# pachterlab/kallisto

Hardware: NVIDIA H100
Metric: paired reads/sec quant (higher is better)
Workload: dtype u64/f64

## Files before the change

kallisto_b200/csrc/kernels_align.cu:

```cuda
#include "kb_device.cuh"
#include "kb_dict.cuh"
#include "kernels.hpp"

#ifndef KB_MATCH_MIN_BLOCKS
#define KB_MATCH_MIN_BLOCKS 3
#endif
#ifdef KB_MATCH_STATS
#include <cstdio>
#endif

namespace kb {

#ifdef KB_MATCH_STATS
enum : int {
  MS_WARP_ITERS, MS_SERVICE_ROUNDS, MS_LANE_ITERS, MS_CHAIN_ITERS,
  MS_MAIN_HIT, MS_MAIN_MISS_FILTER, MS_MAIN_MISS_SLOT, MS_JUMP, MS_MIDDLE, MS_BACKOFF, MS_COLLISION,
  MS_CYCLES_LOOKUP, MS_CYCLES_SERVICE,
  MS_CYCLES_KEY, MS_CYCLES_WAIT, MS_CYCLES_STEP,
  MS_RUN_HIST, MS_N = MS_RUN_HIST + 9
};
__device__ unsigned long long kb_match_stats[MS_N];
static const char* const kMatchStatNames[MS_N] = {
  "warp_iters", "service_rounds", "lane_iters", "chain_iters",
  "main_hit", "main_miss_filter", "main_miss_slot", "jump", "middle", "backoff", "collision",
  "cycles_lookup", "cycles_service", "cycles_key", "cycles_wait", "cycles_step",
  "run_1", "run_2", "run_3", "run_4", "run_5_8", "run_9_16", "run_17_32", "run_33_64", "run_65_"};
__device__ __forceinline__ int run_bin(int n) {
  return n <= 4 ? n - 1 : (n <= 8 ? 4 : (n <= 16 ? 5 : (n <= 32 ? 6 : (n <= 64 ? 7 : 8))));
}
#define KB_MS(i, n) (ms[i] += (unsigned long long)(n))
#define KB_MS_ONLY(x) x
#else
#define KB_MS(i, n) ((void)0)
#define KB_MS_ONLY(x)
#endif

namespace {

__device__ __forceinline__ int32_t ld_relaxed_s32(const int32_t* p) {
  int32_t v;
  asm volatile("ld.relaxed.gpu.global.s32 %0, [%1];" : "=r"(v) : "l"(p) : "memory");
  return v;
}
__device__ __forceinline__ void ld256_nc(const void* p, uint32_t (&w)[8]) {
  asm volatile("ld.global.nc.v4.b32 {%0,%1,%2,%3}, [%8]; ld.global.nc.v4.b32 {%4,%5,%6,%7}, [%8+16];"
               : "=r"(w[0]), "=r"(w[1]), "=r"(w[2]), "=r"(w[3]), "=r"(w[4]), "=r"(w[5]), "=r"(w[6]), "=r"(w[7])
               : "l"(p));
}
struct ReadView {
  const uint32_t* bw;
  const uint32_t* gmask;
  int n_mask;
  int stride;
  int len;
  int k;
  bool has_invalid;

  __device__ __forceinline__ uint64_t kmer(int p) const {
    const int w = p >> 4, s = (p & 15) * 2;
    uint64_t x = (uint64_t)bw[w * stride] << 32;
    if (s + 2 * k > 32) x |= bw[(w + 1) * stride];
    x <<= s;
    if (s + 2 * k > 64) x |= (uint64_t)(bw[(w + 2) * stride] >> (32 - s));
    return x >> (64 - 2 * k);
  }
  __device__ __forceinline__ int next_valid(int p) const {
    if (!has_invalid) return p <= len - k ? p : -1;
    const uint64_t wmask = (1ULL << k) - 1;
    while (p <= len - k) {
      const int w = p >> 5, s = p & 31;
      const uint64_t lo = __ldg(gmask + w);
      const uint64_t hi = (w + 1 < n_mask) ? __ldg(gmask + w + 1) : 0xFFFFFFFFu;
      const uint64_t x = (((hi << 32) | lo) >> s) & wmask;
      if (x == 0) return p;
      p += 64 - __clzll((long long)x);
    }
    return -1;
  }
};

__device__ __forceinline__ uint64_t tuple_hash(const uint32_t* w, int n, int stride) {
  uint64_t h = 0x243F6A8885A308D3ULL ^ (uint64_t)n;
  for (int i = 0; i < n; ++i) h = kb_mix64(h ^ ((uint64_t)w[i * stride] + 0x9E3779B97F4A7C15ULL * (i + 1)));
  return h;
}

__device__ __forceinline__ int32_t memo2_lookup(const DevDict& dd, uint32_t e0, uint32_t e1) {
  const unsigned long long key = ((unsigned long long)e0 << 32) | e1;
  uint64_t s = kb_mix64(key) & dd.m2_mask;
  for (;;) {
    const unsigned long long kk = __ldcg(&dd.m2[s].key);
    if (kk == key) return ld_relaxed_s32(&dd.m2[s].val);
    if (kk == ~0ULL) return KB_H_NOTREADY;
    s = (s + 1) & dd.m2_mask;
  }
}
__device__ __forceinline__ bool tuple_equal(const DevDict& dd, uint32_t toff, const uint32_t* w, int n, int stride) {
  const uint32_t* t = dd.tpool + toff;
  bool eq = __ldcg(t) == (uint32_t)n;
  for (int i = 0; eq && i < n; ++i) eq = __ldcg(t + 1 + i) == w[i * stride];
  return eq;
}
__device__ __forceinline__ int32_t memon_lookup(const DevDict& dd, const uint32_t* w, int n, int stride) {
  const uint64_t th = tuple_hash(w, n, stride);
  const uint32_t tag = (uint32_t)(th >> 32);
  uint64_t s = th & dd.mn_mask;
  for (;;) {
    const unsigned long long word = ld_acquire_u64(&dd.mn_key[s]);
    if (word == ~0ULL) return KB_H_NOTREADY;
    if ((uint32_t)(word >> 32) == tag && tuple_equal(dd, (uint32_t)word, w, n, stride)) return ld_relaxed_s32(&dd.mn_val[s]);
    s = (s + 1) & dd.mn_mask;
  }
}

__device__ __forceinline__ void read_span(const BatchArgs& ba, uint32_t ridx, const uint8_t*& base, uint64_t& off, int& len) {
  base = ba.bases;
  const uint32_t* offs = ba.off;
  uint32_t i = ridx;
  if (ba.bases2) {
    i = ridx >> 1;
    if (ridx & 1) { base = ba.bases2; offs = ba.off2; }
  }
  if (offs) {
    const uint32_t o0 = offs[i], o1 = offs[i + 1];
    off = o0;
    len = (int)(o1 - o0);
  } else {
    off = (uint64_t)i * ba.fixed_len;
    len = (int)ba.fixed_len;
  }
  const bool second = ba.paired && (ridx & 1);
  uint32_t st = second ? ba.start2 : ba.start;
  if (ba.notag && ba.notag[ba.paired ? (ridx >> 1) : ridx]) st = second ? ba.alt_start2 : ba.alt_start;
  if (st) {
    off += st;
    len -= (int)st;
    if (len < 0) len = 0;
  }
  if (ba.skip && ba.skip[ba.paired ? (ridx >> 1) : ridx]) len = 0;
}

enum : int {
  S_MAIN = 0, S_JUMP = 1, S_MIDDLE = 2, S_BACKOFF = 3,
  S_FIN = 4,
  S_EMPTY = 5
};
enum : int { C_BLK = 0, C_DS = 1, C_POS = 2, C_NP = 3, C_H2U = 4, C_H2E = 5, C_P2 = 6, C_P3 = 7, C_DIST = 8, C_HU = 9, C_HE = 10 };
static_assert(C_HE + 1 == KB_CHAIN_WORDS, "match_lane_words counts every cold word of a chain");

}

__global__ void __launch_bounds__(256) pack_kernel(BatchArgs ba, uint32_t n_reads, uint32_t* out) {
  const uint32_t gid = blockIdx.x * blockDim.x + threadIdx.x;
  const uint32_t nb = ba.nb;
  if (gid >= n_reads * nb) return;
  const uint32_t r = gid / nb, w = gid - r * nb;
  uint64_t off;
  int len;
  const uint8_t* src_bases;
  read_span(ba, r, src_bases, off, len);
  const int base = (int)w * 32;
  uint32_t hi = 0, lo = 0, inv32 = ~0u;
  if (base < len) {
    const int n = min(32, len - base);
    const uint64_t a = off + (uint64_t)base;
    const uint32_t* wp = reinterpret_cast<const uint32_t*>(src_bases + (a & ~3ull));
    const int sh = (int)(a & 3) * 8;
    const int last = ((int)(a & 3) + n - 1) >> 2;
    uint32_t wd[9];
#pragma unroll
    for (int q = 0; q < 9; ++q) wd[q] = __ldg(wp + min(q, last));
    uint32_t d[8], pr[8];
#pragma unroll
    for (int q = 0; q < 8; ++q) {
      const uint32_t four = __funnelshift_r(wd[q], wd[q + 1], sh);
      uint32_t x = (four >> 1) & 0x03030303u;
      const uint32_t y = (x | (x >> 4)) & 0x00330033u;
      d[q] = (four & 0xDFDFDFDFu) ^ __byte_perm(0x47544341u, 0u, y | (y >> 8));
      x ^= (x >> 1) & 0x01010101u;
      pr[q] = x * 0x40100401u;
    }
    hi = __byte_perm(__byte_perm(pr[3], pr[2], 0x0073u), __byte_perm(pr[1], pr[0], 0x0073u), 0x5410u);
    lo = __byte_perm(__byte_perm(pr[7], pr[6], 0x0073u), __byte_perm(pr[5], pr[4], 0x0073u), 0x5410u);
    const bool full = (n == 32);
    uint32_t any = full ? (d[0] | d[1] | d[2] | d[3] | d[4] | d[5] | d[6] | d[7]) : 1u;
    inv32 = 0;
    if (any) {
      const int ng = (n + 3) >> 2;
#pragma unroll
      for (int q = 0; q < 8; ++q) {
        if (q >= ng) break;
        uint32_t t = (d[q] & 0x7F7F7F7Fu) + 0x7F7F7F7Fu;
        t = (t | d[q]) & 0x80808080u;
        inv32 |= (((t >> 7) * 0x01020408u) >> 24) << (4 * q);
      }
    }
    if (!full) {
      inv32 |= ~0u << n;
      if (n > 16) lo &= ~0u << (64 - 2 * n);
      else { lo = 0; if (n < 16) hi &= ~0u << (32 - 2 * n); }
    }
  }
  uint32_t* dst = out + (size_t)r * ba.pstride;
  reinterpret_cast<uint2*>(dst)[w] = make_uint2(lo, hi);
  dst[2 * nb + w] = inv32;
  for (uint32_t j = 3 * nb + w; j < ba.pstride; j += nb) dst[j] = ~0u;
}

__global__ void __launch_bounds__(256) dlist_scan_kernel(DevIndex ix, BatchArgs ba, uint32_t n_reads) {
  const uint64_t gid = (uint64_t)blockIdx.x * blockDim.x + threadIdx.x;
  const uint32_t nb = ba.nb;
  if (gid >= (uint64_t)n_reads * nb) return;
  const uint32_t r = (uint32_t)(gid / nb), w = (uint32_t)(gid % nb);
  const uint32_t frag = ba.paired ? (r >> 1) : r;
  uint64_t off;
  int len;
  const uint8_t* unused;
  read_span(ba, r, unused, off, len);
  const int k = ix.k;
  const int p0 = (int)w * 32;
  if (len < k || p0 > len - k) return;
  const uint32_t* pk = ba.packed + (size_t)r * ba.pstride;
  const unsigned long long* bw = reinterpret_cast<const unsigned long long*>(pk);
  const unsigned long long w0 = bw[w], w1 = (w + 1 < nb) ? bw[w + 1] : 0ull;
  const unsigned long long inv = (unsigned long long)pk[2 * nb + w] | ((w + 1 < nb) ? ((unsigned long long)pk[2 * nb + w + 1] << 32) : 0xFFFFFFFF00000000ull);
  const unsigned long long wmask = (1ull << k) - 1;
  for (int j = 0; j < 32; ++j) {
    const int p = p0 + j;
    if (p > len - k) break;
    if ((inv >> j) & wmask) continue;
    unsigned long long x = w0 << (2 * j);
    if (j) x |= w1 >> (64 - 2 * j);
    const uint64_t fwd = x >> (64 - 2 * k);
    const uint64_t rc = kb_revcomp(fwd, k);
    const uint64_t canon = fwd < rc ? fwd : rc;
    uint64_t h = kb_mix64(canon) & ix.dfk_mask;
    for (;;) {
      const unsigned long long key = __ldg(ix.dfk + h);
      if (key == canon) { ba.skip_w[frag] = 1; return; }
      if (key == KB_EMPTY_KEY) break;
      h = (h + 1) & ix.dfk_mask;
    }
  }
}

__global__ void __launch_bounds__(256, KB_MATCH_MIN_BLOCKS) match_kernel(DevIndex ix, DevDict dd, BatchArgs ba) {
  extern __shared__ uint32_t smem[];
  const int tid = threadIdx.x, nt = blockDim.x;
  const unsigned lane = tid & 31;
  const int nb = (int)ba.nb, nw = 2 * nb;
  const int k = ix.k;
  uint32_t* elist = smem + tid;
  uint32_t* cold = elist + (size_t)KB_MAX_E * nt;
  uint32_t* s_bw = cold + (size_t)2 * KB_CHAIN_WORDS * nt;
  uint32_t* spill = ba.spill + ((size_t)blockIdx.x * nt + tid) * KB_SPILL;
  static_assert(C_BLK < C_POS && C_DS < C_POS && C_POS == 2 && C_NP == C_POS + 1 && C_HE == KB_CHAIN_WORDS - 1,
                "a tuple grown by 6 words past KB_MAX_E overwrites exactly the first-hit words of both chains");
  auto cw = [&](int w, int c) -> uint32_t& { return cold[(size_t)(2 * w + c) * nt]; };

  const uint32_t n_warps = (gridDim.x * nt) >> 5;
  const uint32_t gw = (blockIdx.x * nt + tid) >> 5;
  const uint32_t chunk = (ba.n_frag + n_warps - 1) / n_warps;
  uint32_t next = min(ba.n_frag, gw * chunk);
  const uint32_t end = min(ba.n_frag, next + chunk);
  const int n_mates = ba.paired ? 2 : 1;
  const int n_chunks = (int)(ba.pstride >> 3);

  __shared__ unsigned long long s_tot[3];
  if (tid < 3) s_tot[tid] = 0;
  __syncthreads();

  uint32_t frag = 0;
  int n_e = 0;
  bool overflow = false;
  unsigned inv_flags = 0;
  int st[2] = {S_EMPTY, S_EMPTY};
  int p[2] = {-1, -1}, len[2] = {0, 0};
  bool need_prep[2] = {false, false}, is_canon[2] = {false, false};
  bool hv[2] = {false, false}, hs[2] = {false, false};
  uint64_t canon[2] = {0, 0};
  uint32_t slot[2] = {0, 0};
  const uint32_t slot_mask = (uint32_t)ix.mask;
  uint32_t pv = 0;
#ifdef KB_MATCH_STATS
  unsigned long long ms[MS_N] = {};
  int run[2] = {0, 0};
  long long t_mark = clock64();
  long long t_step = -1;
  auto end_run = [&](int c) { if (run[c] > 0) { KB_MS(MS_RUN_HIST + run_bin(run[c]), 1); run[c] = 0; } };
#endif
  auto view = [&](int c) {
    ReadView rv;
    rv.bw = s_bw + (size_t)c * nw * nt;
    rv.gmask = ba.packed + (size_t)(ba.paired ? 2 * frag + c : frag) * ba.pstride + nw;
    rv.n_mask = nb;
    rv.stride = nt;
    rv.len = len[c];
    rv.k = k;
    rv.has_invalid = ((inv_flags >> c) & 1u) != 0;
    return rv;
  };

  KB_MS_ONLY(bool in_service = true;)
  for (;;) {
#ifdef KB_MATCH_STATS
    {
      const long long t_now = clock64();
      KB_MS(in_service ? MS_CYCLES_SERVICE : MS_CYCLES_LOOKUP, t_now - t_mark);
      if (t_step >= 0) KB_MS(MS_CYCLES_STEP, t_now - t_step);
      t_mark = t_now;
      t_step = -1;
    }
#endif
    const bool done = st[0] == S_FIN && st[1] == S_FIN;
    const unsigned fin = __ballot_sync(0xFFFFFFFFu, done);
    const unsigned idle = fin | __ballot_sync(0xFFFFFFFFu, st[0] == S_EMPTY);
    const bool work_left = next < end;
    if (idle == 0xFFFFFFFFu && fin == 0 && !work_left) break;
    KB_MS_ONLY(in_service = false;)
    if (idle == 0xFFFFFFFFu || (work_left && __popc(idle) >= ba.refill_min)) {
      KB_MS(MS_SERVICE_ROUNDS, 1);
      KB_MS_ONLY(in_service = true;)
      if (done) {
        bool memo_hit = false;
        const bool v0 = hv[0], s0 = hs[0], v1 = hv[1], s1 = hs[1];
        uint32_t f_blk[2], f_ds[2], f_pos[2];
#pragma unroll
        for (int c = 0; c < 2; ++c) { f_blk[c] = cw(C_BLK, c); f_ds[c] = cw(C_DS, c); f_pos[c] = cw(C_POS, c); }
        bool mapped = v0 || v1;
        if ((v0 && !s0) || (v1 && !s1)) mapped = false;
        if (mapped && n_e == 0) mapped = false;
        int32_t handle = KB_H_UNMAPPED;
        if (mapped) {
          const bool want_fp = ba.fp_fl >= 0 && (!ba.paired || !v0 || !v1);
          const bool stranded = ba.strand_mode != 0;
          uint32_t xs0 = 0xFFFFFFFFu, xs1 = 0xFFFFFFFFu;
          if (stranded) {
            xs0 = v0 ? (f_blk[0] * 2u + (f_ds[0] >> 31)) : 0xFFFFFFFFu;
            xs1 = v1 ? (f_blk[1] * 2u + (f_ds[1] >> 31)) : 0xFFFFFFFFu;
            if (ba.notag && ba.notag[frag]) xs0 = xs1 = 0xFFFFFFFFu;
          }
          const uint32_t x_blk = v1 ? f_blk[1] : f_blk[0], x_ds = v1 ? f_ds[1] : f_ds[0], x_pos = v1 ? f_pos[1] : f_pos[0];
          const uint32_t xf0 = x_blk;
          const uint32_t xf1 = x_ds >> 31;
          const uint32_t xf2 = x_pos;
          const uint32_t xf3 = x_ds & 0x7FFFFFFFu;
          const int nx = (stranded ? 2 : 0) + (want_fp ? 4 : 0);
          auto put_extras = [&](uint32_t* dst, int at, int st) {
            if (stranded) { dst[at * st] = xs0; dst[(at + 1) * st] = xs1; at += 2; }
            if (want_fp) { dst[at * st] = xf0; dst[(at + 1) * st] = xf1; dst[(at + 2) * st] = xf2; dst[(at + 3) * st] = xf3; }
          };
          if (overflow) {
            atomicOr(dd.error, KB_DEVERR_E_OVERFLOW);
          } else if (n_e > KB_MAX_E) {
            auto E = [&](int i) -> uint32_t { return i < KB_MAX_E ? elist[i * nt] : spill[i - KB_MAX_E]; };
            auto S = [&](int i, uint32_t x) { if (i < KB_MAX_E) elist[i * nt] = x; else spill[i - KB_MAX_E] = x; };
            for (int i = 1; i < n_e; ++i) {
              const uint32_t x = E(i);
              int j = i - 1;
              while (j >= 0 && E(j) > x) { S(j + 1, E(j)); --j; }
              S(j + 1, x);
            }
            const uint32_t q = atomicAdd(ba.qbig_count, 1u);
            if (q >= ba.qbig_cap) {
              atomicOr(dd.error, KB_DEVERR_E_OVERFLOW);
            } else {
              uint32_t* e = ba.qbig_entries + (size_t)q * KB_QBIG_STRIDE;
              e[0] = frag;
              e[1] = (uint32_t)(n_e + nx) | (want_fp ? 0x80000000u : 0u) | 0x40000000u;
              for (int i = 0; i < n_e; ++i) e[2 + i] = E(i);
              put_extras(e + 2, n_e, 1);
              handle = KB_H_PENDING;
            }
          } else {
            for (int i = 1; i < n_e; ++i) {
              const uint32_t x = elist[i * nt];
              int j = i - 1;
              while (j >= 0 && elist[j * nt] > x) { elist[(j + 1) * nt] = elist[j * nt]; --j; }
              elist[(j + 1) * nt] = x;
            }
            if (ba.strand_mode == 0 && n_e == 1 && !want_fp) {
              handle = (int32_t)elist[0];
            } else {
              const int n = n_e + nx;
              int32_t r;
              if (ba.strand_mode == 0 && n_e == 2 && !want_fp) {
                r = memo2_lookup(dd, elist[0], elist[nt]);
              } else {
                put_extras(elist, n_e, nt);
                r = want_fp ? KB_H_NOTREADY : memon_lookup(dd, elist, n, nt);
              }
              if (r == KB_H_NOTREADY) {
                handle = KB_H_PENDING;
                const uint32_t q = atomicAdd(ba.q_count, 1u);
                uint32_t* e = ba.q_entries + (size_t)q * KB_Q_STRIDE;
                e[0] = frag;
                e[1] = (uint32_t)n | (want_fp ? 0x80000000u : 0u);
                for (int i = 0; i < n; ++i) e[2 + i] = elist[i * nt];
              } else {
                handle = r;
                memo_hit = true;
              }
            }
          }
        }
        ba.handle_out[frag] = handle;
        if (ba.tl_out) {
          uint16_t tl = 0;
          if (ba.paired && v0 && v1) {
            int q[2];
            bool strand[2];
#pragma unroll
            for (int c = 0; c < 2; ++c) {
              const int d = (int)(f_ds[c] & 0x7FFFFFFFu);
              strand[c] = (f_ds[c] >> 31) != 0;
              q[c] = strand[c] ? d - (int)f_pos[c] : d + k + (int)f_pos[c];
            }
            if (f_blk[0] == f_blk[1] && strand[0] != strand[1]) {
              const int d = q[0] > q[1] ? q[0] - q[1] : q[1] - q[0];
              if (d > 0 && d < 1000) tl = (uint16_t)d;
            }
          }
          if (ba.notag && !ba.notag[frag]) tl = 0;
          ba.tl_out[frag] = tl;
        }
        if (ba.first_hit) ba.first_hit[frag] = v0 ? f_blk[0] * 2u + (f_ds[0] >> 31) : 0xFFFFFFFFu;
        const unsigned grp = __match_any_sync(fin, handle);
        const uint32_t fmin = __reduce_min_sync(grp, frag);
        if (handle >= 0 && !ba.no_count && lane == (unsigned)(__ffs(grp) - 1)) {
          atomicAdd(&dd.count[handle], (uint32_t)__popc(grp));
          atomicMin(&dd.first[handle], (unsigned long long)(ba.frag_base + fmin));
        }
        const uint32_t r_probes = __reduce_add_sync(fin, pv & 0xFFFFu), r_visits = __reduce_add_sync(fin, pv >> 16);
        const uint32_t r_memo = __popc(__ballot_sync(fin, memo_hit));
        pv = 0;
        if (lane == (unsigned)(__ffs(fin) - 1)) {
          atomicAdd(&s_tot[0], (unsigned long long)r_probes);
          atomicAdd(&s_tot[1], (unsigned long long)r_visits);
          if (r_memo) atomicAdd(&s_tot[2], (unsigned long long)r_memo);
        }
        st[0] = st[1] = S_EMPTY;
      }
      __syncwarp();
      {
        const bool is_idle = (idle >> lane) & 1u;
        const uint32_t rank = __popc(idle & ((1u << lane) - 1));
        const uint32_t avail = end - next;
        if (is_idle && rank < avail) {
          const uint32_t fidx = next + rank;
          unsigned inv = 0;
#pragma unroll
          for (int mt = 0; mt < 2; ++mt) {
            len[mt] = 0;
            if (mt >= n_mates) continue;
            const uint32_t ridx = ba.paired ? 2 * fidx + mt : fidx;
            const uint8_t* unused_base;
            uint64_t unused_off;
            int l;
            read_span(ba, ridx, unused_base, unused_off, l);
            if (l > nb * 32) l = nb * 32;
            len[mt] = l;
            const uint32_t* src = ba.packed + (size_t)ridx * ba.pstride;
            uint32_t* dbw = s_bw + (size_t)mt * nw * nt;
            uint32_t bad = 0;
            for (int c = 0; c < n_chunks; ++c) {
              uint32_t v[8];
              ld256_nc(src + c * 8, v);
#pragma unroll
              for (int i = 0; i < 8; ++i) {
                const int g = c * 8 + i;
                if (g < nw) {
                  dbw[(g ^ 1) * nt] = v[i];
                } else if (g < nw + nb) {
                  const int first = (g - nw) * 32;
                  const uint32_t in_read = l >= first + 32 ? 0xFFFFFFFFu : (l > first ? ((1u << (l - first)) - 1u) : 0u);
                  bad |= v[i] & in_read;
                }
              }
            }
            if (bad) inv |= 1u << mt;
          }
          frag = fidx;
          n_e = 0;
          overflow = false;
          inv_flags = inv;
#pragma unroll
          for (int c = 0; c < 2; ++c) {
            hv[c] = hs[c] = false;
            need_prep[c] = true;
            st[c] = S_FIN;
            if (c < n_mates) {
              p[c] = view(c).next_valid(0);
              if (p[c] >= 0) st[c] = S_MAIN;
            }
          }
        }
        const uint32_t n_idle = __popc(idle);
        next += n_idle < avail ? n_idle : avail;
      }
      continue;
    }
    const bool live[2] = {st[0] <= S_BACKOFF, st[1] <= S_BACKOFF};
    KB_MS(MS_WARP_ITERS, 1);
    if (live[0] || live[1]) {
      KB_MS(MS_LANE_ITERS, 1);
      uint32_t fword[2] = {0xFFFFFFFFu, 0xFFFFFFFFu}, fbit[2] = {0, 0};
#pragma unroll
      for (int c = 0; c < 2; ++c) {
        if (live[c] && need_prep[c]) {
          const bool filtered = st[c] == S_MAIN || st[c] == S_BACKOFF;
          const int pq = filtered ? p[c] : (int)cw(st[c] == S_JUMP ? C_P2 : C_P3, c);
          const uint64_t fwd = view(c).kmer(pq);
          const uint64_t rc = kb_revcomp(fwd, k);
          is_canon[c] = fwd < rc;
          canon[c] = is_canon[c] ? fwd : rc;
          const uint64_t hsh = kb_mix64(canon[c]);
          slot[c] = (uint32_t)hsh & slot_mask;
          need_prep[c] = false;
          ++pv;
          if (ix.filter && filtered) {
            const uint32_t fidx = (uint32_t)(hsh >> 32) & ix.filter_mask;
            fword[c] = __ldg(ix.filter + (fidx >> 5));
            fbit[c] = fidx & 31;
          }
        }
      }
#ifdef KB_MATCH_STATS
      const long long t_key = clock64();
#endif
      uint32_t v[2][8];
#pragma unroll
      for (int c = 0; c < 2; ++c) {
        if (live[c] && ((fword[c] >> fbit[c]) & 1u)) {
          ld256_nc(ix.slots + slot[c], v[c]);
          pv += 0x10000u;
        } else {
          v[c][0] = v[c][1] = 0xFFFFFFFFu;
        }
      }
#ifdef KB_MATCH_STATS
      {
        long long t_wait = t_key;
        if (((v[0][0] ^ v[0][1]) ^ 3u * (v[1][0] ^ v[1][1])) != 0x0BADF00Du) t_wait = clock64();
        KB_MS(MS_CYCLES_KEY, t_key - t_mark);
        KB_MS(MS_CYCLES_WAIT, t_wait - t_key);
        t_step = t_wait;
      }
#endif
#pragma unroll
      for (int c = 0; c < 2; ++c) {
        if (!live[c]) continue;
        KB_MS(MS_CHAIN_ITERS, 1);
        const uint64_t key = (uint64_t)v[c][0] | ((uint64_t)v[c][1] << 32);
        if (key != canon[c] && key != KB_EMPTY_KEY) {
          slot[c] = (slot[c] + 1) & slot_mask;
          KB_MS(MS_COLLISION, 1);
          continue;
        }
        const bool f = key == canon[c];
#ifdef KB_MATCH_STATS
        if (st[c] == S_MAIN) {
          if (f) { KB_MS(MS_MAIN_HIT, 1); end_run(c); }
          else { KB_MS(((fword[c] >> fbit[c]) & 1u) ? MS_MAIN_MISS_SLOT : MS_MAIN_MISS_FILTER, 1); ++run[c]; }
        } else {
          KB_MS(st[c] == S_JUMP ? MS_JUMP : (st[c] == S_MIDDLE ? MS_MIDDLE : MS_BACKOFF), 1);
        }
#endif
        const uint32_t r_unitig = v[c][2], r_ec = v[c][4];
        const bool r_strand = (is_canon[c] == ((v[c][5] >> 31) != 0));
        const int l = len[c];
        const ReadView rv = view(c);
        bool push = false, end_chain = false, to_backoff = false;
        int nv_from = -1;
        if (st[c] == S_MAIN) {
          if (!f) {
            nv_from = p[c] + 1;
          } else {
            push = true;
            const int r_dist = (int)(v[c][5] & 0x7FFFFFFFu);
            const int off = r_dist - (int)v[c][6], blen = (int)(v[c][7] - v[c][6]);
            const int dist = r_strand ? (blen - 1 - off) : off;
            if (dist >= 2) {
              const int np = (p[c] + dist >= l - k) ? (l - k) : (p[c] + dist);
              const int p2 = rv.next_valid(np);
              if (p2 < 0) {
                end_chain = true;
              } else {
                cw(C_NP, c) = (uint32_t)np;
                cw(C_P2, c) = (uint32_t)p2;
                cw(C_DIST, c) = (uint32_t)dist;
                cw(C_HU, c) = r_unitig; cw(C_HE, c) = r_ec;
                st[c] = S_JUMP;
                need_prep[c] = true;
              }
            } else {
              nv_from = p[c] + 1;
            }
          }
        } else if (st[c] == S_JUMP) {
          const bool found2 = !f || (cw(C_HU, c) == r_unitig && cw(C_HE, c) == r_ec);
          const int dist = (int)cw(C_DIST, c);
          const int found2pos = !f ? p[c] : p[c] + dist;
          if (found2) {
            if (found2pos >= l - k) end_chain = true;
            else nv_from = (int)cw(C_P2, c) + 1;
          } else {
            cw(C_H2U, c) = r_unitig; cw(C_H2E, c) = r_ec;
            if (dist > 4) {
              const int middlePos = (p[c] + (int)cw(C_NP, c)) / 2;
              const int p3 = rv.next_valid(middlePos);
              if (p3 >= 0) { cw(C_P3, c) = (uint32_t)p3; st[c] = S_MIDDLE; need_prep[c] = true; }
              else to_backoff = true;
            } else {
              to_backoff = true;
            }
          }
        } else if (st[c] == S_MIDDLE) {
          const bool foundMiddle = f && ((cw(C_HU, c) == r_unitig && cw(C_HE, c) == r_ec) ||
                                         (cw(C_H2U, c) == r_unitig && cw(C_H2E, c) == r_ec));
          if (foundMiddle) {
            push = true;
            if ((int)cw(C_NP, c) >= l - k) end_chain = true;
            else nv_from = (int)cw(C_P2, c) + 1;
          } else {
            to_backoff = true;
          }
        } else {
          push = f;
          nv_from = p[c] + 1;
        }
        if (push) {
          if (!hv[c]) {
            hv[c] = true;
            cw(C_BLK, c) = v[c][3];
            cw(C_DS, c) = (v[c][5] & 0x7FFFFFFFu) | (r_strand ? 0x80000000u : 0u);
            cw(C_POS, c) = (uint32_t)p[c];
          }
          if (r_ec != ba.empty_ec) {
            hs[c] = true;
            bool dup = false;
            const int n_sh = n_e < KB_MAX_E ? n_e : KB_MAX_E;
            for (int i = 0; i < n_sh; ++i) dup |= (elist[i * nt] == r_ec);
            for (int i = KB_MAX_E; i < n_e; ++i) dup |= (spill[i - KB_MAX_E] == r_ec);
            if (!dup) {
              if (n_e < KB_MAX_E) { elist[n_e * nt] = r_ec; ++n_e; }
              else if (n_e < KB_MAX_E + KB_SPILL) { spill[n_e - KB_MAX_E] = r_ec; ++n_e; }
              else overflow = true;
            }
          }
        }
        if (to_backoff) nv_from = p[c] + 1;
        if (nv_from >= 0) {
          p[c] = rv.next_valid(nv_from);
          if (p[c] < 0) end_chain = true;
          else { st[c] = to_backoff ? S_BACKOFF : S_MAIN; need_prep[c] = true; }
        }
        if (end_chain) st[c] = S_FIN;
        KB_MS_ONLY(if (st[c] == S_FIN) end_run(c);)
      }
    }
  }
  __syncthreads();
  if (tid < 3 && s_tot[tid]) atomicAdd(&dd.stats[tid == 0 ? 0 : (tid == 1 ? 3 : 2)], s_tot[tid]);
#ifdef KB_MATCH_STATS
  for (int i = 0; i < MS_N; ++i) {
    const bool per_warp = i == MS_WARP_ITERS || i == MS_SERVICE_ROUNDS || i == MS_CYCLES_LOOKUP || i == MS_CYCLES_SERVICE;
    unsigned long long x = ms[i];
    if (!per_warp)
      for (int o = 16; o > 0; o >>= 1) x += __shfl_xor_sync(0xFFFFFFFFu, x, o);
    if (lane == 0 && x) atomicAdd(&kb_match_stats[i], x);
  }
#endif
}

template <int G>
__global__ void __launch_bounds__(128, 8) resolve_kernel(DevIndex ix, DevDict dd, BatchArgs ba, ResolveArgs ra) {
  const unsigned lane = threadIdx.x & (G - 1);
  const unsigned gmask = group_mask<G>(threadIdx.x & 31);
  const unsigned gshift = (threadIdx.x & 31) & ~(unsigned)(G - 1);
  const uint32_t warp = (blockIdx.x * blockDim.x + threadIdx.x) / G;
  if (warp >= ra.n_warps) return;
  uint32_t* scratch = ra.scratch + (size_t)warp * ra.scratch_stride;
  const uint32_t* pool = dd.pool;

  for (int pass = 0; pass < 2; ++pass) {
  const uint32_t nq = pass == 0 ? *ba.q_count : min(*ba.qbig_count, ba.qbig_cap);
  const uint32_t* entries = pass == 0 ? ba.q_entries : ba.qbig_entries;
  const size_t stride = pass == 0 ? (size_t)KB_Q_STRIDE : (size_t)KB_QBIG_STRIDE;
  if (warp == 0 && lane == 0 && nq) atomicAdd(&dd.stats[1], (unsigned long long)nq);
  for (uint32_t q = warp; q < nq; q += ra.n_warps) {
    const uint32_t* e = entries + (size_t)q * stride;
    const uint32_t f = e[0];
    const bool has_fp = (e[1] >> 31) != 0;
    const bool no_memo = has_fp || ((e[1] >> 30) & 1u) != 0;
    const int n = (int)(e[1] & 0xFFFFu);
    const uint32_t* w = e + 2;
    const bool stranded = ba.strand_mode != 0;
    const int n_e = n - (stranded ? 2 : 0) - (has_fp ? 4 : 0);
    const bool use_m2 = (!stranded && !no_memo && n_e == 2);

    int32_t handle = KB_H_NOTREADY;
    if (lane == 0 && !no_memo) handle = use_m2 ? memo2_lookup(dd, w[0], w[1]) : memon_lookup(dd, w, n, 1);
    handle = __shfl_sync(gmask, handle, 0, G);

    if (handle == KB_H_NOTREADY) {
      int sm = 0;
      uint32_t sm_len = (uint32_t)((dd.dslots[w[0]] >> 32) & 0xFFFFFFu);
      for (int j = 1; j < n_e; ++j) {
        const uint32_t len = (uint32_t)((dd.dslots[w[j]] >> 32) & 0xFFFFFFu);
        if (len < sm_len) { sm_len = len; sm = j; }
      }
      const uint32_t* A = pool + (uint32_t)dd.dslots[w[sm]];
      uint32_t nres = 0;
      for (uint32_t base = 0; base < sm_len; base += G) {
        const uint32_t i = base + lane;
        bool alive = i < sm_len;
        const uint32_t a = alive ? __ldcg(A + i) : 0;
        for (int j = 0; j < n_e; ++j) {
          if (j == sm) continue;
          const unsigned long long bw_ = dd.dslots[w[j]];
          const uint32_t* B = pool + (uint32_t)bw_;
          const uint32_t blen = (uint32_t)((bw_ >> 32) & 0xFFFFFFu);
          if (alive) alive = bsearch_contains(B, blen, a, nullptr);
        }
        const unsigned bal = (__ballot_sync(gmask, alive) >> gshift);
        if (alive) scratch[nres + __popc(bal & ((1u << lane) - 1))] = a;
        nres += __popc(bal);
      }
      __syncwarp(gmask);
      if (has_fp && nres > 0) {
        const uint32_t* fw = w + n - 4;
        const uint32_t blk = fw[0];
        const bool csense = fw[1] != 0;
        const long long pp = (long long)fw[2], udist = (long long)fw[3];
        const long long usize = (long long)ix.blk_usize[blk], kk = (long long)ix.k, fl = (long long)ba.fp_fl;
        const unsigned long long bword = dd.dslots[ix.blk_ec[blk]];
        const uint32_t* B = pool + (uint32_t)bword;
        const uint32_t blen = (uint32_t)((bword >> 32) & 0xFFFFFFu);
        const uint4* info = ix.fp_info + ix.blk_strand_off[blk];
        uint32_t n_v = 0;
        for (uint32_t base = 0; base < nres; base += G) {
          const uint32_t i = base + lane;
          bool keep = false;
          const uint32_t tr = i < nres ? scratch[i] : 0;
          if (i < nres) {
            uint32_t rank = 0;
            if (bsearch_contains(B, blen, tr, &rank)) {
              const uint4 c = info[rank];
              const long long trpos = (long long)(c.x & 0x7FFFFFFFu);
              const bool trsense = (c.x >> 31) == 0;
              long long x;
              bool s;
              if (trsense) {
                if (csense) { x = trpos - pp + udist + 1 - (long long)c.y; s = true; }
                else { x = trpos + pp + kk + udist - (long long)c.z; s = false; }
              } else {
                if (csense) { x = trpos - udist + usize - (long long)c.w + pp; s = false; }
                else { x = trpos + usize - udist - (long long)c.w - kk + 1 - pp; s = true; }
              }
              const int xi = (int)x;
              keep = (s && xi + (int)fl <= (int)ix.target_len[tr]) || (!s && xi - (int)fl >= 0);
            }
          }
          const unsigned bv = (__ballot_sync(gmask, keep) >> gshift);
          if (keep) scratch[ra.scratch_stride / 2 + n_v + __popc(bv & ((1u << lane) - 1))] = tr;
          n_v += __popc(bv);
        }
        __syncwarp(gmask);
        if (n_v < nres) {
          for (uint32_t i = lane; i < n_v; i += G) scratch[i] = scratch[ra.scratch_stride / 2 + i];
          nres = n_v;
        }
        __syncwarp(gmask);
      }
      if (stranded) {
        for (int mate = 0; mate < 2 && nres > 0; ++mate) {
          const uint32_t sw = w[n_e + mate];
          if (sw == 0xFFFFFFFFu) continue;
          const uint32_t blk = sw >> 1;
          const bool um_strand = (sw & 1) != 0;
          const bool want = (mate == 0) ? (ba.strand_mode == 1) : (ba.strand_mode == 2);
          const unsigned long long bword = dd.dslots[ix.blk_ec[blk]];
          const uint32_t* B = pool + (uint32_t)bword;
          const uint32_t blen = (uint32_t)((bword >> 32) & 0xFFFFFFu);
          const uint8_t* sb = ix.strand + ix.blk_strand_off[blk];
          uint32_t n_u = 0, n_v = 0;
          for (uint32_t base = 0; base < nres; base += G) {
            const uint32_t i = base + lane;
            bool in_u = i < nres;
            const uint32_t a = in_u ? scratch[i] : 0;
            uint32_t rank = 0;
            if (in_u) in_u = bsearch_contains(B, blen, a, &rank);
            bool in_v = false;
            if (in_u) {
              const uint8_t sense = sb[rank];
              in_v = ((um_strand == (sense != 0)) == want) || sense == 2;
            }
            const unsigned bu = (__ballot_sync(gmask, in_u) >> gshift);
            const unsigned bv = (__ballot_sync(gmask, in_v) >> gshift);
            __syncwarp(gmask);
            if (in_u) scratch[n_u + __popc(bu & ((1u << lane) - 1))] = a;
            if (in_v) scratch[ra.scratch_stride / 2 + n_v + __popc(bv & ((1u << lane) - 1))] = a;
            n_u += __popc(bu);
            n_v += __popc(bv);
            __syncwarp(gmask);
          }
          if (n_v < n_u) {
            for (uint32_t i = lane; i < n_v; i += G) scratch[i] = scratch[ra.scratch_stride / 2 + i];
            nres = n_v;
          } else {
            nres = n_u;
          }
          __syncwarp(gmask);
        }
      }
      handle = nres == 0 ? KB_H_UNMAPPED : dict_insert_warp<G>(dd, scratch, nres, lane, gmask);
      if (lane == 0 && !no_memo) {
        if (use_m2) {
          const unsigned long long key = ((unsigned long long)w[0] << 32) | w[1];
          uint64_t s = kb_mix64(key) & dd.m2_mask;
          uint64_t visited = 0;
          for (;;) {
            const unsigned long long old = atomicCAS(&dd.m2[s].key, ~0ULL, key);
            if (old == ~0ULL || old == key) { atomicExch(&dd.m2[s].val, handle); break; }
            s = (s + 1) & dd.m2_mask;
            if (++visited > dd.m2_mask) { atomicOr(dd.error, KB_DEVERR_MEMO_FULL); break; }
          }
        } else {
          const uint64_t th = tuple_hash(w, n, 1);
          const uint32_t tag = (uint32_t)(th >> 32);
          const unsigned long long toff = atomicAdd(dd.tpool_top, (unsigned long long)(n + 1));
          if (toff + n + 1 > dd.tpool_cap) {
            atomicOr(dd.error, KB_DEVERR_TPOOL_FULL);
          } else {
            dd.tpool[toff] = (uint32_t)n;
            for (int i = 0; i < n; ++i) dd.tpool[toff + 1 + i] = w[i];
            __threadfence();
            const unsigned long long word = ((unsigned long long)tag << 32) | toff;
            uint64_t s = th & dd.mn_mask;
            uint64_t visited = 0;
            for (;;) {
              unsigned long long old = atomicCAS(&dd.mn_key[s], ~0ULL, word);
              bool mine = (old == ~0ULL);
              if (!mine && (uint32_t)(old >> 32) == tag) {
                const uint32_t* t = dd.tpool + (uint32_t)old;
                bool eq = __ldcg(t) == (uint32_t)n;
                for (int i = 0; eq && i < n; ++i) eq = __ldcg(t + 1 + i) == w[i];
                mine = eq;
              }
              if (mine) { atomicExch(&dd.mn_val[s], handle); break; }
              s = (s + 1) & dd.mn_mask;
              if (++visited > dd.mn_mask) { atomicOr(dd.error, KB_DEVERR_MEMO_FULL); break; }
            }
          }
        }
      }
    }
    if (lane == 0) {
      ba.handle_out[f] = handle;
      if (handle >= 0 && !ba.no_count) {
        atomicAdd(&dd.count[handle], 1u);
        atomicMin(&dd.first[handle], (unsigned long long)(ba.frag_base + f));
      }
    }
    __syncwarp(gmask);
  }
  }
}

__global__ void fld_finalize_kernel(DevDict dd, BatchArgs ba) {
  const uint32_t f = blockIdx.x * blockDim.x + threadIdx.x;
  if (f >= ba.n_frag) return;
  const int32_t h = ba.handle_out[f];
  if (h < 0) { ba.tl_out[f] = 0; return; }
  const unsigned long long word = dd.dslots[h];
  if (((word >> 32) & 0xFFFFFFu) != 1) ba.tl_out[f] = 0;
}

__global__ void collect_used_kernel(DevDict dd, uint32_t* used, uint32_t* n_used) {
  const uint64_t stride = (uint64_t)gridDim.x * blockDim.x;
  for (uint64_t h = (uint64_t)blockIdx.x * blockDim.x + threadIdx.x; h <= dd.dmask; h += stride) {
    if (dd.count[h] > 0) used[atomicAdd(n_used, 1u)] = (uint32_t)h;
  }
}

void launch_pseudoalign(const DevIndex& ix, const DevDict& dd, const BatchArgs& ba, const ResolveArgs& ra,
                        int tpb, cudaStream_t st, cudaEvent_t* ev) {
  if (ba.n_frag == 0) return;
  cudaMemsetAsync(ba.q_count, 0, sizeof(uint32_t), st);
  cudaMemsetAsync(ba.qbig_count, 0, sizeof(uint32_t), st);
  const size_t smem = (size_t)tpb * 4 * match_lane_words(ba.nb);
  const int sms = device_sm_count();
  cudaFuncSetAttribute(match_kernel, cudaFuncAttributeMaxDynamicSharedMemorySize, (int)smem);
  int per_sm = 0;
  cudaOccupancyMaxActiveBlocksPerMultiprocessor(&per_sm, match_kernel, tpb, smem);
  if (per_sm < 1) per_sm = 1;
  unsigned blocks = (unsigned)(sms * per_sm);
  const unsigned need = (ba.n_frag + tpb - 1) / tpb;
  if (blocks > need) blocks = need;
  if (ev) cudaEventRecord(ev[0], st);
  {
    const uint32_t n_reads = ba.paired ? 2 * ba.n_frag : ba.n_frag;
    const uint64_t total = (uint64_t)n_reads * ba.nb;
    pack_kernel<<<(unsigned)((total + 255) / 256), 256, 0, st>>>(ba, n_reads, const_cast<uint32_t*>(ba.packed));
    if (ix.dfk && ba.skip_w) dlist_scan_kernel<<<(unsigned)((total + 255) / 256), 256, 0, st>>>(ix, ba, n_reads);
  }
  if (ev) cudaEventRecord(ev[1], st);
#ifdef KB_MATCH_STATS
  void* ms_dev = nullptr;
  cudaGetSymbolAddress(&ms_dev, kb_match_stats);
  cudaMemsetAsync(ms_dev, 0, sizeof(unsigned long long) * MS_N, st);
#endif
  match_kernel<<<blocks, tpb, smem, st>>>(ix, dd, ba);
#ifdef KB_MATCH_STATS
  {
    unsigned long long h[MS_N];
    cudaMemcpyAsync(h, ms_dev, sizeof(h), cudaMemcpyDeviceToHost, st);
    cudaStreamSynchronize(st);
    fprintf(stderr, "kb_match_stats {\"n_frag\": %u", ba.n_frag);
    for (int i = 0; i < MS_N; ++i) fprintf(stderr, ", \"%s\": %llu", kMatchStatNames[i], h[i]);
    fprintf(stderr, "}\n");
  }
#endif
  if (ev) cudaEventRecord(ev[2], st);
  switch (ra.group) {
    case 4: resolve_kernel<4><<<(ra.n_warps * 4 + 127) / 128, 128, 0, st>>>(ix, dd, ba, ra); break;
    case 8: resolve_kernel<8><<<(ra.n_warps * 8 + 127) / 128, 128, 0, st>>>(ix, dd, ba, ra); break;
    case 16: resolve_kernel<16><<<(ra.n_warps * 16 + 127) / 128, 128, 0, st>>>(ix, dd, ba, ra); break;
    default: resolve_kernel<32><<<(ra.n_warps * 32 + 127) / 128, 128, 0, st>>>(ix, dd, ba, ra); break;
  }
  if (ev) cudaEventRecord(ev[3], st);
}

__global__ void __launch_bounds__(128) import_sets_kernel(DevDict dd, uint32_t n_sets, const uint32_t* off, const uint32_t* tids,
                                                         const uint32_t* counts, const unsigned long long* first,
                                                         unsigned long long first_offset) {
  const unsigned lane = threadIdx.x & 31;
  const uint32_t w = (blockIdx.x * blockDim.x + threadIdx.x) >> 5;
  const uint32_t nw = (gridDim.x * blockDim.x) >> 5;
  for (uint32_t s = w; s < n_sets; s += nw) {
    const uint32_t o0 = off[s], n = off[s + 1] - o0;
    if (n == 0) continue;
    const int32_t h = dict_insert_warp(dd, tids + o0, n, lane);
    if (lane == 0 && h >= 0) {
      atomicAdd(&dd.count[h], counts[s]);
      atomicMin(&dd.first[h], first[s] + first_offset);
    }
    __syncwarp();
  }
}

struct ImportSegs {
  int n;
  uint32_t prefix[KB_IMPORT_SEGS + 1];
  ImportSeg seg[KB_IMPORT_SEGS];
};
__global__ void __launch_bounds__(128) import_segments_kernel(DevDict dd, ImportSegs a) {
  const unsigned lane = threadIdx.x & 31;
  const uint32_t w = (blockIdx.x * blockDim.x + threadIdx.x) >> 5;
  const uint32_t nw = (gridDim.x * blockDim.x) >> 5;
  const uint32_t total = a.prefix[a.n];
  for (uint32_t g = w; g < total; g += nw) {
    int k = 0;
    while (g >= a.prefix[k + 1]) ++k;
    const ImportSeg& sg = a.seg[k];
    const uint32_t s = g - a.prefix[k];
    const uint32_t o0 = sg.off[s], n = sg.off[s + 1] - o0;
    if (n == 0) continue;
    const int32_t h = dict_insert_warp(dd, sg.tids + o0, n, lane);
    if (lane == 0 && h >= 0) {
      atomicAdd(&dd.count[h], sg.counts[s]);
      atomicMin(&dd.first[h], sg.first[s]);
    }
    __syncwarp();
  }
}

int device_sm_count() {
  static int sms[64] = {0};
  int dev = 0;
  cudaGetDevice(&dev);
  if (dev < 0 || dev >= 64) dev = 0;
  if (sms[dev] == 0) {
    int v = 0;
    cudaDeviceGetAttribute(&v, cudaDevAttrMultiProcessorCount, dev);
    sms[dev] = v > 0 ? v : 1;
  }
  return sms[dev];
}

void launch_import_segments(const DevDict& dd, const ImportSeg* segs, int n_segs, cudaStream_t st) {
  if (n_segs <= 0) return;
  ImportSegs a;
  a.n = n_segs;
  a.prefix[0] = 0;
  for (int i = 0; i < n_segs; ++i) { a.seg[i] = segs[i]; a.prefix[i + 1] = a.prefix[i] + segs[i].n_sets; }
  if (a.prefix[n_segs] == 0) return;
  const unsigned warps_needed = a.prefix[n_segs];
  unsigned blocks = (unsigned)device_sm_count() * 16;
  if (blocks > (warps_needed + 3) / 4) blocks = (warps_needed + 3) / 4;
  import_segments_kernel<<<blocks, 128, 0, st>>>(dd, a);
}

void launch_import_sets(const DevDict& dd, uint32_t n_sets, const uint32_t* off, const uint32_t* tids, const uint32_t* counts,
                        const unsigned long long* first, unsigned long long first_offset, cudaStream_t st) {
  if (n_sets == 0) return;
  import_sets_kernel<<<device_sm_count() * 8, 128, 0, st>>>(dd, n_sets, off, tids, counts, first, first_offset);
}

void launch_fld_finalize(const DevDict& dd, const BatchArgs& ba, cudaStream_t st) {
  if (ba.n_frag == 0 || !ba.tl_out) return;
  fld_finalize_kernel<<<(ba.n_frag + 255) / 256, 256, 0, st>>>(dd, ba);
}

void launch_collect_used(const DevDict& dd, uint32_t* used, uint32_t* n_used, cudaStream_t st) {
  cudaMemsetAsync(n_used, 0, sizeof(uint32_t), st);
  collect_used_kernel<<<device_sm_count() * 8, 256, 0, st>>>(dd, used, n_used);
}

}
```

Before: 440.1 million.

## Roll k-mers incrementally and split match step into fast straight path plus generic pass

Keeps forward and reverse-complement k-mers per mate and updates them by one base when the next query position is adjacent, instead of re-extracting and reverse-complementing the whole k-mer. Hash collisions and plain MAIN misses on valid reads now take a cheap straight-line path. Other state transitions go through a serialized generic pass over a todo mask, with the state machine code emitted only once instead of unrolled per mate. This aims to cut per-step ALU work and code size, at the cost of more live registers (fwd/rc pairs) and a dependent while loop that can serialize mates.

```diff
diff --git a/kallisto_b200/csrc/kernels_align.cu b/kallisto_b200/csrc/kernels_align.cu
--- a/kallisto_b200/csrc/kernels_align.cu
+++ b/kallisto_b200/csrc/kernels_align.cu
@@ -17,13 +17,14 @@
   MS_MAIN_HIT, MS_MAIN_MISS_FILTER, MS_MAIN_MISS_SLOT, MS_JUMP, MS_MIDDLE, MS_BACKOFF, MS_COLLISION,
   MS_CYCLES_LOOKUP, MS_CYCLES_SERVICE,
   MS_CYCLES_KEY, MS_CYCLES_WAIT, MS_CYCLES_STEP,
+  MS_STRAIGHT, MS_GEN_PASSES,
   MS_RUN_HIST, MS_N = MS_RUN_HIST + 9
 };
 __device__ unsigned long long kb_match_stats[MS_N];
 static const char* const kMatchStatNames[MS_N] = {
   "warp_iters", "service_rounds", "lane_iters", "chain_iters",
   "main_hit", "main_miss_filter", "main_miss_slot", "jump", "middle", "backoff", "collision",
-  "cycles_lookup", "cycles_service", "cycles_key", "cycles_wait", "cycles_step",
+  "cycles_lookup", "cycles_service", "cycles_key", "cycles_wait", "cycles_step", "straight", "gen_passes",
   "run_1", "run_2", "run_3", "run_4", "run_5_8", "run_9_16", "run_17_32", "run_33_64", "run_65_"};
 __device__ __forceinline__ int run_bin(int n) {
   return n <= 4 ? n - 1 : (n <= 8 ? 4 : (n <= 16 ? 5 : (n <= 32 ? 6 : (n <= 64 ? 7 : 8))));
@@ -144,6 +145,11 @@
   S_MAIN = 0, S_JUMP = 1, S_MIDDLE = 2, S_BACKOFF = 3,
   S_FIN = 4,
   S_EMPTY = 5
+};
+enum : int {
+  P_NONE = 0,
+  P_BUILD = 1,
+  P_ROLL = 2
 };
 enum : int { C_BLK = 0, C_DS = 1, C_POS = 2, C_NP = 3, C_H2U = 4, C_H2E = 5, C_P2 = 6, C_P3 = 7, C_DIST = 8, C_HU = 9, C_HE = 10 };
 static_assert(C_HE + 1 == KB_CHAIN_WORDS, "match_lane_words counts every cold word of a chain");
@@ -276,11 +282,12 @@
   unsigned inv_flags = 0;
   int st[2] = {S_EMPTY, S_EMPTY};
   int p[2] = {-1, -1}, len[2] = {0, 0};
-  bool need_prep[2] = {false, false}, is_canon[2] = {false, false};
-  bool hv[2] = {false, false}, hs[2] = {false, false};
-  uint64_t canon[2] = {0, 0};
+  int prep[2] = {P_NONE, P_NONE};
+  unsigned hv = 0, hs = 0;
+  uint64_t fwd[2] = {0, 0}, rc[2] = {0, 0};
   uint32_t slot[2] = {0, 0};
   const uint32_t slot_mask = (uint32_t)ix.mask;
+  const uint64_t kmask = (1ULL << (2 * k)) - 1;
   uint32_t pv = 0;
 #ifdef KB_MATCH_STATS
   unsigned long long ms[MS_N] = {};
@@ -289,13 +296,13 @@
   long long t_step = -1;
   auto end_run = [&](int c) { if (run[c] > 0) { KB_MS(MS_RUN_HIST + run_bin(run[c]), 1); run[c] = 0; } };
 #endif
-  auto view = [&](int c) {
+  auto view = [&](int c, int l) {
     ReadView rv;
     rv.bw = s_bw + (size_t)c * nw * nt;
     rv.gmask = ba.packed + (size_t)(ba.paired ? 2 * frag + c : frag) * ba.pstride + nw;
     rv.n_mask = nb;
     rv.stride = nt;
-    rv.len = len[c];
+    rv.len = l;
     rv.k = k;
     rv.has_invalid = ((inv_flags >> c) & 1u) != 0;
     return rv;
@@ -323,7 +330,7 @@
       KB_MS_ONLY(in_service = true;)
       if (done) {
         bool memo_hit = false;
-        const bool v0 = hv[0], s0 = hs[0], v1 = hv[1], s1 = hs[1];
+        const bool v0 = hv & 1u, s0 = hs & 1u, v1 = hv & 2u, s1 = hs & 2u;
         uint32_t f_blk[2], f_ds[2], f_pos[2];
 #pragma unroll
         for (int c = 0; c < 2; ++c) { f_blk[c] = cw(C_BLK, c); f_ds[c] = cw(C_DS, c); f_pos[c] = cw(C_POS, c); }
@@ -484,13 +491,13 @@
           n_e = 0;
           overflow = false;
           inv_flags = inv;
+          hv = hs = 0;
 #pragma unroll
           for (int c = 0; c < 2; ++c) {
-            hv[c] = hs[c] = false;
-            need_prep[c] = true;
+            prep[c] = P_BUILD;
             st[c] = S_FIN;
             if (c < n_mates) {
-              p[c] = view(c).next_valid(0);
+              p[c] = view(c, len[c]).next_valid(0);
               if (p[c] >= 0) st[c] = S_MAIN;
             }
           }
@@ -502,21 +509,27 @@
     }
     const bool live[2] = {st[0] <= S_BACKOFF, st[1] <= S_BACKOFF};
     KB_MS(MS_WARP_ITERS, 1);
+    KB_MS_ONLY(int n_pass = 0;)
     if (live[0] || live[1]) {
       KB_MS(MS_LANE_ITERS, 1);
       uint32_t fword[2] = {0xFFFFFFFFu, 0xFFFFFFFFu}, fbit[2] = {0, 0};
 #pragma unroll
       for (int c = 0; c < 2; ++c) {
-        if (live[c] && need_prep[c]) {
+        if (live[c] && prep[c] != P_NONE) {
           const bool filtered = st[c] == S_MAIN || st[c] == S_BACKOFF;
-          const int pq = filtered ? p[c] : (int)cw(st[c] == S_JUMP ? C_P2 : C_P3, c);
-          const uint64_t fwd = view(c).kmer(pq);
-          const uint64_t rc = kb_revcomp(fwd, k);
-          is_canon[c] = fwd < rc;
-          canon[c] = is_canon[c] ? fwd : rc;
-          const uint64_t hsh = kb_mix64(canon[c]);
+          if (prep[c] == P_ROLL) {
+            const int q = p[c] + k - 1;
+            const uint64_t b = (s_bw[((size_t)c * nw + (q >> 4)) * nt] >> (30 - 2 * (q & 15))) & 3u;
+            fwd[c] = ((fwd[c] << 2) | b) & kmask;
+            rc[c] = (rc[c] >> 2) | ((b ^ 3u) << (2 * k - 2));
+          } else {
+            const int pq = filtered ? p[c] : (int)cw(st[c] == S_JUMP ? C_P2 : C_P3, c);
+            fwd[c] = view(c, len[c]).kmer(pq);
+            rc[c] = kb_revcomp(fwd[c], k);
+          }
+          const uint64_t hsh = kb_mix64(fwd[c] < rc[c] ? fwd[c] : rc[c]);
           slot[c] = (uint32_t)hsh & slot_mask;
-          need_prep[c] = false;
+          prep[c] = P_NONE;
           ++pv;
           if (ix.filter && filtered) {
             const uint32_t fidx = (uint32_t)(hsh >> 32) & ix.filter_mask;
@@ -547,41 +560,66 @@
         t_step = t_wait;
       }
 #endif
+      bool f[2];
+      unsigned todo = 0;
 #pragma unroll
       for (int c = 0; c < 2; ++c) {
-        if (!live[c]) continue;
-        KB_MS(MS_CHAIN_ITERS, 1);
         const uint64_t key = (uint64_t)v[c][0] | ((uint64_t)v[c][1] << 32);
-        if (key != canon[c] && key != KB_EMPTY_KEY) {
-          slot[c] = (slot[c] + 1) & slot_mask;
-          KB_MS(MS_COLLISION, 1);
-          continue;
-        }
-        const bool f = key == canon[c];
+        f[c] = key == (fwd[c] < rc[c] ? fwd[c] : rc[c]);
+        const bool coll = live[c] && !f[c] && key != KB_EMPTY_KEY;
+        const bool step = live[c] && !f[c] && !coll && st[c] == S_MAIN && !((inv_flags >> c) & 1u);
 #ifdef KB_MATCH_STATS
-        if (st[c] == S_MAIN) {
-          if (f) { KB_MS(MS_MAIN_HIT, 1); end_run(c); }
-          else { KB_MS(((fword[c] >> fbit[c]) & 1u) ? MS_MAIN_MISS_SLOT : MS_MAIN_MISS_FILTER, 1); ++run[c]; }
-        } else {
-          KB_MS(st[c] == S_JUMP ? MS_JUMP : (st[c] == S_MIDDLE ? MS_MIDDLE : MS_BACKOFF), 1);
-        }
-#endif
-        const uint32_t r_unitig = v[c][2], r_ec = v[c][4];
-        const bool r_strand = (is_canon[c] == ((v[c][5] >> 31) != 0));
-        const int l = len[c];
-        const ReadView rv = view(c);
+        if (live[c]) {
+          KB_MS(MS_CHAIN_ITERS, 1);
+          if (coll || step) KB_MS(MS_STRAIGHT, 1);
+          if (coll) {
+            KB_MS(MS_COLLISION, 1);
+          } else if (st[c] == S_MAIN) {
+            if (f[c]) { KB_MS(MS_MAIN_HIT, 1); end_run(c); }
+            else { KB_MS(((fword[c] >> fbit[c]) & 1u) ? MS_MAIN_MISS_SLOT : MS_MAIN_MISS_FILTER, 1); ++run[c]; }
+          } else {
+            KB_MS(st[c] == S_JUMP ? MS_JUMP : (st[c] == S_MIDDLE ? MS_MIDDLE : MS_BACKOFF), 1);
+          }
+        }
+#endif
+        if (coll) slot[c] = (slot[c] + 1) & slot_mask;
+        if (step) {
+          ++p[c];
+          prep[c] = P_ROLL;
+          if (p[c] > len[c] - k) st[c] = S_FIN;
+          KB_MS_ONLY(if (st[c] == S_FIN) end_run(c);)
+        }
+        if (live[c] && !coll && !step) todo |= 1u << c;
+      }
+      while (todo) {
+        KB_MS_ONLY(++n_pass;)
+        const bool c1 = !(todo & 1u);
+        const int c = c1 ? 1 : 0;
+        todo &= todo - 1;
+        const int s = c1 ? st[1] : st[0];
+        const int pc = c1 ? p[1] : p[0];
+        const int l = c1 ? len[1] : len[0];
+        const bool fc = c1 ? f[1] : f[0];
+        const bool is_canon = c1 ? fwd[1] < rc[1] : fwd[0] < rc[0];
+        uint32_t h[6];
+#pragma unroll
+        for (int i = 0; i < 6; ++i) h[i] = c1 ? v[1][i + 2] : v[0][i + 2];
+        const uint32_t r_unitig = h[0], r_ec = h[2];
+        const bool r_strand = (is_canon == ((h[3] >> 31) != 0));
+        const ReadView rv = view(c, l);
+        int ns = s, np_ = pc, npr = P_BUILD;
         bool push = false, end_chain = false, to_backoff = false;
         int nv_from = -1;
-        if (st[c] == S_MAIN) {
-          if (!f) {
-            nv_from = p[c] + 1;
+        if (s == S_MAIN) {
+          if (!fc) {
+            nv_from = pc + 1;
           } else {
             push = true;
-            const int r_dist = (int)(v[c][5] & 0x7FFFFFFFu);
-            const int off = r_dist - (int)v[c][6], blen = (int)(v[c][7] - v[c][6]);
+            const int r_dist = (int)(h[3] & 0x7FFFFFFFu);
+            const int off = r_dist - (int)h[4], blen = (int)(h[5] - h[4]);
             const int dist = r_strand ? (blen - 1 - off) : off;
             if (dist >= 2) {
-              const int np = (p[c] + dist >= l - k) ? (l - k) : (p[c] + dist);
+              const int np = (pc + dist >= l - k) ? (l - k) : (pc + dist);
               const int p2 = rv.next_valid(np);
               if (p2 < 0) {
                 end_chain = true;
@@ -590,34 +628,33 @@
                 cw(C_P2, c) = (uint32_t)p2;
                 cw(C_DIST, c) = (uint32_t)dist;
                 cw(C_HU, c) = r_unitig; cw(C_HE, c) = r_ec;
-                st[c] = S_JUMP;
-                need_prep[c] = true;
+                ns = S_JUMP;
               }
             } else {
-              nv_from = p[c] + 1;
-            }
-          }
-        } else if (st[c] == S_JUMP) {
-          const bool found2 = !f || (cw(C_HU, c) == r_unitig && cw(C_HE, c) == r_ec);
+              nv_from = pc + 1;
+            }
+          }
+        } else if (s == S_JUMP) {
+          const bool found2 = !fc || (cw(C_HU, c) == r_unitig && cw(C_HE, c) == r_ec);
           const int dist = (int)cw(C_DIST, c);
-          const int found2pos = !f ? p[c] : p[c] + dist;
+          const int found2pos = !fc ? pc : pc + dist;
           if (found2) {
             if (found2pos >= l - k) end_chain = true;
             else nv_from = (int)cw(C_P2, c) + 1;
           } else {
             cw(C_H2U, c) = r_unitig; cw(C_H2E, c) = r_ec;
             if (dist > 4) {
-              const int middlePos = (p[c] + (int)cw(C_NP, c)) / 2;
+              const int middlePos = (pc + (int)cw(C_NP, c)) / 2;
               const int p3 = rv.next_valid(middlePos);
-              if (p3 >= 0) { cw(C_P3, c) = (uint32_t)p3; st[c] = S_MIDDLE; need_prep[c] = true; }
+              if (p3 >= 0) { cw(C_P3, c) = (uint32_t)p3; ns = S_MIDDLE; }
               else to_backoff = true;
             } else {
               to_backoff = true;
             }
           }
-        } else if (st[c] == S_MIDDLE) {
-          const bool foundMiddle = f && ((cw(C_HU, c) == r_unitig && cw(C_HE, c) == r_ec) ||
-                                         (cw(C_H2U, c) == r_unitig && cw(C_H2E, c) == r_ec));
+        } else if (s == S_MIDDLE) {
+          const bool foundMiddle = fc && ((cw(C_HU, c) == r_unitig && cw(C_HE, c) == r_ec) ||
+                                          (cw(C_H2U, c) == r_unitig && cw(C_H2E, c) == r_ec));
           if (foundMiddle) {
             push = true;
             if ((int)cw(C_NP, c) >= l - k) end_chain = true;
@@ -626,18 +663,18 @@
             to_backoff = true;
           }
         } else {
-          push = f;
-          nv_from = p[c] + 1;
+          push = fc;
+          nv_from = pc + 1;
         }
         if (push) {
-          if (!hv[c]) {
-            hv[c] = true;
-            cw(C_BLK, c) = v[c][3];
-            cw(C_DS, c) = (v[c][5] & 0x7FFFFFFFu) | (r_strand ? 0x80000000u : 0u);
-            cw(C_POS, c) = (uint32_t)p[c];
+          if (!((hv >> c) & 1u)) {
+            hv |= 1u << c;
+            cw(C_BLK, c) = h[1];
+            cw(C_DS, c) = (h[3] & 0x7FFFFFFFu) | (r_strand ? 0x80000000u : 0u);
+            cw(C_POS, c) = (uint32_t)pc;
           }
           if (r_ec != ba.empty_ec) {
-            hs[c] = true;
+            hs |= 1u << c;
             bool dup = false;
             const int n_sh = n_e < KB_MAX_E ? n_e : KB_MAX_E;
             for (int i = 0; i < n_sh; ++i) dup |= (elist[i * nt] == r_ec);
@@ -649,22 +686,29 @@
             }
           }
         }
-        if (to_backoff) nv_from = p[c] + 1;
+        if (to_backoff) nv_from = pc + 1;
         if (nv_from >= 0) {
-          p[c] = rv.next_valid(nv_from);
-          if (p[c] < 0) end_chain = true;
-          else { st[c] = to_backoff ? S_BACKOFF : S_MAIN; need_prep[c] = true; }
-        }
-        if (end_chain) st[c] = S_FIN;
-        KB_MS_ONLY(if (st[c] == S_FIN) end_run(c);)
-      }
-    }
+          const int key_pos = (s == S_MAIN || s == S_BACKOFF) ? pc : (int)cw(s == S_JUMP ? C_P2 : C_P3, c);
+          np_ = rv.next_valid(nv_from);
+          if (np_ < 0) end_chain = true;
+          else { ns = to_backoff ? S_BACKOFF : S_MAIN; npr = np_ == key_pos + 1 ? P_ROLL : P_BUILD; }
+        }
+        if (end_chain) ns = S_FIN;
+        KB_MS_ONLY(if (ns == S_FIN) end_run(c);)
+        if (c1) { st[1] = ns; p[1] = np_; prep[1] = npr; }
+        else { st[0] = ns; p[0] = np_; prep[0] = npr; }
+      }
+    }
+#ifdef KB_MATCH_STATS
+    KB_MS(MS_GEN_PASSES, __reduce_max_sync(0xFFFFFFFFu, n_pass));
+#endif
   }
   __syncthreads();
   if (tid < 3 && s_tot[tid]) atomicAdd(&dd.stats[tid == 0 ? 0 : (tid == 1 ? 3 : 2)], s_tot[tid]);
 #ifdef KB_MATCH_STATS
   for (int i = 0; i < MS_N; ++i) {
-    const bool per_warp = i == MS_WARP_ITERS || i == MS_SERVICE_ROUNDS || i == MS_CYCLES_LOOKUP || i == MS_CYCLES_SERVICE;
+    const bool per_warp = i == MS_WARP_ITERS || i == MS_SERVICE_ROUNDS || i == MS_CYCLES_LOOKUP || i == MS_CYCLES_SERVICE ||
+                          i == MS_GEN_PASSES;
     unsigned long long x = ms[i];
     if (!per_warp)
       for (int o = 16; o > 0; o >>= 1) x += __shfl_xor_sync(0xFFFFFFFFu, x, o);
```

Result: faster. 457.2 million (median of 6 runs) (+3.9%).
